# Scthe/cnn-Super-Resolution

Measured on AMD Instinct MI355X. Metric: training tiles/sec (fwd+bwd+update), default SRCNN 33x33, batch 4096/GPU, higher is better.
Workload: dtype f32

## Files before the change

cnn-super-resolution_amd/csrc/hip/d1x6.hpp:

```cpp

constexpr int kD6Mxx = 12, kD6Mx3 = 25;
constexpr int kD6ExWin = 6, kD6ExMid = 3;
constexpr int kD6Grow = 70;

constexpr int kD6Zero = 32;
__device__ __attribute__((aligned(16))) float g_d6_zero[kD6Zero] = {};
constexpr int d6_row_half(bool d3, int h) { return (d3 ? 4 : 8) * h; }
constexpr int d6_zero_half(bool d3, int h) { return d6_row_half(d3, h); }
constexpr int d6_row_quad(bool d3, int k) { return d3 ? 8 * k : 16 * (k >> 1) + 4 * (k & 1); }
constexpr bool d6_zero_row_covers(bool d3) {
  for (int h = 0; h < 2; h++)
    for (int k = 0; k < 4; k++)
      if (d6_zero_half(d3, h) + d6_row_quad(d3, k) + 4 > kD6Zero) return false;
  return true;
}

__device__ __forceinline__ void mma_x6_2(const bf16x8 (&a0)[3], const bf16x8 (&b0)[3], f32x16& c0,
                                         const bf16x8 (&a1)[3], const bf16x8 (&b1)[3], f32x16& c1) {
  using mfma::mma_bf16;
  c0 = mma_bf16(a0[2], b0[0], c0);
  c1 = mma_bf16(a1[2], b1[0], c1);
  c0 = mma_bf16(a0[1], b0[1], c0);
  c1 = mma_bf16(a1[1], b1[1], c1);
  c0 = mma_bf16(a0[0], b0[2], c0);
  c1 = mma_bf16(a1[0], b1[2], c1);
  c0 = mma_bf16(a0[1], b0[0], c0);
  c1 = mma_bf16(a1[1], b1[0], c1);
  c0 = mma_bf16(a0[0], b0[1], c0);
  c1 = mma_bf16(a1[0], b1[1], c1);
  c0 = mma_bf16(a0[0], b0[0], c0);
  c1 = mma_bf16(a1[0], b1[0], c1);
}

__device__ __forceinline__ void d6_split(const float (&v)[8], bf16x8 (&o)[3]) { mfma::split8(v, o); }

template <bool kD3, bool kTr = false>
__global__ __launch_bounds__(256, 1) void d1x6_grad12_kernel(const float* __restrict__ X,
                                                              const float* __restrict__ A1T,
                                                              const float* __restrict__ D2,
                                                              const float* __restrict__ A2,
                                                              const uint32_t* __restrict__ M2,
                                                              const float* __restrict__ W2,
                                                              const float* __restrict__ W3,
                                                              float* __restrict__ slab, Geom g, RunGeom rg,
                                                              D3Geom dg) {
  constexpr int N1 = 64, N2 = 32, F1 = 9, K1 = F1 * F1;
  constexpr int NW1 = K1 * N1, NW2 = N1 * N2, P12 = NW1 + N1 + NW2 + N2;
  extern __shared__ __attribute__((aligned(16))) float smem[];
  static_assert(kD3 || !kTr, "the part images belong to the delta3 form");
  const D6Lds L(g.W, g.H, rg, kD3);
  char* const base = reinterpret_cast<char*>(smem);
  __bf16* const w2i = reinterpret_cast<__bf16*>(base + L.w2);
  uint32_t* const u32 = reinterpret_cast<uint32_t*>(smem);
  uint32_t* const xbuf = u32 + L.xb / 4;
  int* const slots = reinterpret_cast<int*>(base + L.slots);
  int* const runs = reinterpret_cast<int*>(base + L.runs);

  SRCNN_CLOCK_BEGIN();
  const int lane = mfma::lane_id(), wave = mfma::wave_id();
  const int h = lane >> 5, li = lane & 31;
  const int W = g.W, xn = g.W * g.H, npx = g.ow * g.oh, nch = rg.nch;
  const int x0col = 4 * rg.a;

  float xr[kL12Regs];
  auto xload = [&](int smp) {
    const float* src = X + (size_t)smp * xn;
#pragma unroll
    for (int k = 0; k < kL12Regs; k++) {
      const int i = threadIdx.x + 256 * k;
      xr[k] = i < xn ? src[i] : 0.0f;
    }
  };
  if ((int)blockIdx.x < g.batch) xload(blockIdx.x);

  if constexpr (!kTr)
    for (int i = threadIdx.x; i < nch * 32; i += 256) slots[i] = slot_pixel(rg, i >> 5, i & 31);
  for (int k = threadIdx.x; k < nch * 8; k += 256) {
    int iy, ix;
    bool col;
    run_origin(rg, k < rg.nrun ? k : 0, iy, ix, col);
    runs[(k & ~7) + 4 * (k & 1) + 2 * ((k >> 2) & 1) + ((k >> 1) & 1)] =
        col ? ~(L.rdw + 3 * ((ix - x0col) * L.st + iy)) : 3 * (iy * L.rs + ix);
  }
  for (int i = threadIdx.x; i < (2 * L.xbuf + 3) / 4; i += 256) reinterpret_cast<uint4*>(xbuf)[i] = uint4{0u, 0u, 0u, 0u};
  if (threadIdx.x < 32 && (!kD3 || threadIdx.x < kD6Mxx || (threadIdx.x >= 16 && threadIdx.x < kD6Mx3)))
    u32[L.cst / 4 + threadIdx.x] = !kD3 && (threadIdx.x == 0 || threadIdx.x == 6) ? 0x3F803F80u : 0u;
  {
    constexpr int kIt = 2 * 2 * 64 * 8 / 256;
    float v[kIt];
#pragma unroll
    for (int k = 0; k < kIt; k++) {
      const int e = threadIdx.x + 256 * k;
      const int j = e & 7, L_ = (e >> 3) & 63, kk = (e >> 9) & 1, t = e >> 10;
      const int n = kD3 ? crow(8 * kk + j, L_ >> 5) : 16 * kk + 8 * (L_ >> 5) + j;
      v[k] = W2[(32 * t + (L_ & 31)) * N2 + n];
    }
#pragma unroll
    for (int k = 0; k < kIt; k++) {
      const int e = threadIdx.x + 256 * k;
      const int j = e & 7, L_ = (e >> 3) & 63, kk = (e >> 9) & 1, t = e >> 10;
      __bf16 p[3];
      split3(v[k], p[0], p[1], p[2]);
#pragma unroll
      for (int q = 0; q < 3; q++) w2i[((t * 2 + kk) * 3 + q) * 512 + L_ * 8 + j] = p[q];
    }
  }

  uint32_t* const d3u = u32 + L.d3img / 4;
  const int nout3 = dg.w3 * dg.h3;
  float d3n[2] = {0.0f, 0.0f};
  auto d3load = [&](int smp) {
#pragma unroll
    for (int k = 0; k < 2; k++) {
      const int t = threadIdx.x + 256 * k;
      d3n[k] = t < nout3 ? D2[(size_t)smp * nout3 + t] : 0.0f;
    }
  };
  auto d3build = [&](int buf) {
    uint16_t* const b16 = reinterpret_cast<uint16_t*>(d3u + buf * L.d3buf);
#pragma unroll
    for (int k = 0; k < 2; k++) {
      const int t = threadIdx.x + 256 * k;
      if (t < nout3) {
        const int y = t / dg.w3, x = t - y * dg.w3, d = (y + 5) * L.gs + x + 7;
        __bf16 p[3];
        split3(d3n[k], p[0], p[1], p[2]);
#pragma unroll
        for (int q = 0; q < 3; q++) {
          const uint16_t b = __builtin_bit_cast(uint16_t, p[q]);
          b16[2 * (d + L.gw * q)] = b;
          b16[2 * (d + L.gw * q) - 1] = b;
        }
      }
    }
  };
  float* const mxx = smem + L.cst / 4 + kD6Mxx;
  float* const mx3 = smem + L.cst / 4 + kD6Mx3;
  auto wave_max = [&](float v) {
#pragma unroll
    for (int o = 32; o > 0; o >>= 1) v = fmaxf(v, __shfl_xor(v, o, 64));
    return v;
  };
  auto put_max = [&](float* slot, float v) {
    v = wave_max(v);
    if (lane == 0) slot[wave] = v;
  };
  auto take_max_reg = [&](float v) {
    return __builtin_bit_cast(float, __builtin_amdgcn_readfirstlane(__builtin_bit_cast(int, v)));
  };
  auto take_max = [&](const float* slot) {
    const float v = fmaxf(fmaxf(slot[0], slot[1]), fmaxf(slot[2], slot[3]));
    return __builtin_bit_cast(float, __builtin_amdgcn_readfirstlane(__builtin_bit_cast(int, v)));
  };
  float m3cur = 0.0f, wnorm = 0.0f;
  int EW = 0, EB = 0, EWmin = 1 << 20, EBmin = 1 << 20;
  if constexpr (kD3) {
    {
      float n2 = 0.0f, n3 = 0.0f;
      for (int n = 0; n < N2; n++) n2 += fabsf(W2[lane * N2 + n]);
      for (int t = 0; t < dg.f3 * dg.f3; t++) n3 += fabsf(W3[t * N2 + li]);
      wnorm = take_max_reg(wave_max(n2)) * take_max_reg(wave_max(n3));
    }
    __bf16* const w3i = reinterpret_cast<__bf16*>(base + L.w3i);
    constexpr int kW3It = 2 * 64 * 8 / 256;
    static_assert(kW3It * 256 * 3 == kD6W3, "the W3 image: 2 k-steps x 3 parts");
    float w3v[kW3It];
#pragma unroll
    for (int k = 0; k < kW3It; k++) {
      const int e = threadIdx.x + 256 * k;
      const int j = e & 7, L_ = (e >> 3) & 63, s_ = e >> 9;
      const D3Pair tp = d3_pair_slot(8 * s_ + 4 * (L_ >> 5) + (j >> 1), dg.f3);
      const int dx = d3_pair_dx(tp, j & 1, dg.f3), n = L_ & 31;
      const bool in = dx >= 0;
      w3v[k] = W3[in ? (tp.dy * dg.f3 + dx) * N2 + n : 0];
      if (!in) w3v[k] = 0.0f;
    }
#pragma unroll
    for (int k = 0; k < kW3It; k++) {
      const int e = threadIdx.x + 256 * k;
      const int j = e & 7, L_ = (e >> 3) & 63, s_ = e >> 9;
      __bf16 p[3];
      split3(w3v[k], p[0], p[1], p[2]);
#pragma unroll
      for (int q = 0; q < 3; q++) w3i[((s_ * 3 + q) * 64 + L_) * 8 + j] = p[q];
    }
    int* const d3tab = reinterpret_cast<int*>(base + L.d3tab);
    for (int i = threadIdx.x; i < nch * 32; i += 256) {
      int iy, ix;
      slot_coord(rg, i >> 5, i & 31, iy, ix);
      d3tab[i] = kTr ? d6_slot_pack(slot_pixel(rg, i >> 5, i & 31), iy * L.gs + ix) : iy * L.gs + ix;
    }
    for (int i = threadIdx.x; i < (3 * L.d3buf + 3) / 4; i += 256)
      reinterpret_cast<uint4*>(d3u)[i] = uint4{0u, 0u, 0u, 0u};
    if ((int)blockIdx.x < g.batch) d3load(blockIdx.x);
    put_max(mx3, fmaxf(fabsf(d3n[0]), fabsf(d3n[1])));
    __syncthreads();
    m3cur = take_max(mx3);
    d3build(0);
    if ((int)blockIdx.x + (int)gridDim.x < g.batch) d3load(blockIdx.x + gridDim.x);
  }

  int offR3[3], offT3[3];
#pragma unroll
  for (int u = 0; u < 3; u++) {
    const int tap = 32 * u + li;
    const int dy = tap < K1 ? tap / F1 : 0, dx = tap < K1 ? tap - dy * F1 : 0;
    offR3[u] = 12 * (dy * L.rs + dx);
    offT3[u] = 12 * (dx * L.st + dy);
  }
  typedef __attribute__((address_space(3))) const uint32_t lds_u32;
  const int lds0 = (int)(uintptr_t)(__attribute__((address_space(3))) char*)base;
  const int spec = li == K1 - 64 ? lds0 + L.cst : li > K1 - 64 ? lds0 + L.cst + 64 : -1;

  f32x16 g1[2][3], g2[2];
#pragma unroll
  for (int t = 0; t < 2; t++) {
    g2[t] = zero16();
#pragma unroll
    for (int u = 0; u < 3; u++) g1[t][u] = zero16();
  }
  float gb2 = 0.0f;
  float gbr[16];
#pragma unroll
  for (int r = 0; r < 16; r++) gbr[r] = 0.0f;

  float* const sc = smem + L.sc / 4 + wave * kD6Sc;
  char* const trw = base + L.sc + d6tr_wave_off(wave);
  char* const trw0 = trw + d6tr_write_off(li, h, 0, 0, 0);
  char* const trw1 = trw + d6tr_write_off(li, h, 1, 0, 0);
  const char* const trr = trw + d6tr_read_off(lane, 0, 0, 0);
  const uint16_t* const wl2 = reinterpret_cast<const uint16_t*>(w2i) + lane * 8;

  const float inv_nch = 1.0f / (float)nch;
  auto item = [&](int i, int& j, int& c) {
    j = run_div(i, inv_nch);
    c = i - j * nch;
  };
  auto item_sample = [&](int j) {
    const int smp = (int)blockIdx.x + j * (int)gridDim.x;
    return smp < g.batch ? smp : (int)blockIdx.x;
  };
  f32x4 d2r[4], a1r[2][4];
  uint32_t d2m = 0, d2raw = 0;
  int d2pix = 0;
  auto ld_d2 = [&](int j, int c, int sv) {
    const int pix = kTr ? d6_slot_pix(sv) : slots[c * 32 + li];
    if constexpr (kD3) {
      d2pix = pix;
      d2raw = M2[(size_t)item_sample(j) * npx + (pix >= 0 ? pix : 0)];
    } else {
      static_assert(d6_zero_row_covers(false), "dummy-slot loads past g_d6_zero");
      const float* d2 = pix >= 0 ? D2 + ((size_t)item_sample(j) * npx + pix) * N2 + d6_row_half(false, h)
// ... 118 lines not shown
#pragma unroll
    for (int r = 0; r < 16; r++) {
      const float v = acc[0][r] + acc[1][r];
      d2v[r] = mask_d2(r, v);
    }
  };

  bf16x8 w2k0[2][3];
  auto w2read0 = [&]() __attribute__((always_inline)) {
#pragma unroll
    for (int q = 0; q < 3; q++) {
      w2k0[0][q] = *reinterpret_cast<const bf16x8*>(wl2 + ((0 * 2 + 0) * 3 + q) * 512);
      w2k0[1][q] = *reinterpret_cast<const bf16x8*>(wl2 + ((1 * 2 + 0) * 3 + q) * 512);
    }
  };

  int ki = wave, kj, kc;
  item(ki, kj, kc);
  __syncthreads();
  w2read0();
  {
    const int sv = kD3 ? d3tab_[kc * 32 + li] : 0;
    ld_d2(kj, kc, sv);
    ld_a1(kj, kc);
    if constexpr (kD3) {
      bf16x8 ga[3], gb[3];
      const int t = kTr ? d6_slot_off(sv) : sv;
      d3read(kj, t, 0, ga, gb);
      d2gemm(kj, t, ga, gb);
    } else {
      take_rows();
    }
  }
  if constexpr (kTr) {
    sum_d2(1.0f);
#pragma unroll
    for (int k = 0; k < 2; k++) {
      split_d2(1 + k);
      tr_write(k);
    }
    __builtin_amdgcn_wave_barrier();
    tr_read(0);
    tr_read(1);
  } else {
    stage_d2();
#pragma unroll
    for (int piece = 0; piece < 5; piece++) split_d2(piece);
  }

  for (int it = 0; (int)blockIdx.x + it * (int)gridDim.x < g.batch; it++) {
    const int smp = blockIdx.x + it * gridDim.x;
    uint32_t* const xi = xbuf + (it & 1) * L.xbuf;
    float s1 = 1.0f, sX = 1.0f;
    float m3next = 0.0f;
    if constexpr (kD3) {
      float xm = 0.0f;
#pragma unroll
      for (int k = 0; k < kL12Regs; k++) xm = fmaxf(xm, fabsf(xr[k]));
      float dm = fmaxf(fabsf(d3n[0]), fabsf(d3n[1]));
#pragma unroll
      for (int o = 32; o > 0; o >>= 1) {
        const float tx = __shfl_xor(xm, o, 64), td = __shfl_xor(dm, o, 64);
        xm = fmaxf(xm, tx);
        dm = fmaxf(dm, td);
      }
      if (lane == 0) {
        mxx[wave] = xm;
        mx3[wave] = dm;
      }
      if (smp + (int)gridDim.x < g.batch) d3build((it + 1) - 3 * ((it + 1) / 3));
      __syncthreads();
      const float xmax = take_max(mxx);
      m3next = take_max(mx3);
      const float bound = m3cur * wnorm;
      int e1 = mfma::scale_exp_h(bound), exn = mfma::scale_exp_h(xmax), ex = 0, kb = 0, dW = 0, dB = 0;
      if (exn < mfma::kScaleMin + kD6ExMid) exn = mfma::kScaleMin + kD6ExMid;
      if (bound > 0.0f) {
        int exc = e1 + exn - kD6ExMid - (EWmin + kD6Grow);
        if (exc < e1 - (EBmin + kD6Grow)) exc = e1 - (EBmin + kD6Grow);
        if (exc > 0) e1 = e1 - exc < mfma::kScaleMin ? mfma::kScaleMin : e1 - exc;
        kb = EB - e1;
        if (kb < -14 || kb > 15) {
          dB = e1 - EB;
          EB = e1;
          kb = 0;
        }
        if (xmax > 0.0f) {
          ex = EW - e1;
          if (ex > exn || ex < exn - kD6ExWin) {
            ex = exn - kD6ExMid;
            dW = e1 + ex - EW;
            EW = e1 + ex;
          }
        }
        if (EW < EWmin) EWmin = EW;
        if (EB < EBmin) EBmin = EB;
      } else {
        e1 = 0;
        ex = xmax > 0.0f ? exn - kD6ExMid : 0;
      }
      s1 = mfma::pow2_h(e1);
      sX = mfma::pow2_h(ex);
      if (threadIdx.x == 0) {
        const uint32_t c = (uint32_t)(kb + 15) << 10;
        u32[L.cst / 4 + 3 * (it & 1)] = u32[L.cst / 4 + 3 * (it & 1) + 6] = c | (c << 16);
      }
      while (dW != 0 || dB != 0) {
        const int a = dW < -120 ? -120 : dW > 120 ? 120 : dW, b = dB < -120 ? -120 : dB > 120 ? 120 : dB;
        const float fw = mfma::pow2_h(a), fb = li == K1 - 64 ? mfma::pow2_h(b) : fw;
#pragma unroll
        for (int t = 0; t < 2; t++)
#pragma unroll
          for (int u = 0; u < 3; u++) {
            const float f = u == 2 ? fb : fw;
#pragma unroll
            for (int r = 0; r < 16; r++) g1[t][u][r] *= f;
            __builtin_amdgcn_sched_barrier(0);
          }
        dW -= a;
        dB -= b;
      }
    }
    if constexpr (kD3) {
      uint16_t* const x16 = reinterpret_cast<uint16_t*>(xi);
#pragma unroll
      for (int k = 0; k < kL12Regs; k++) {
        const int i = threadIdx.x + 256 * k;
        if (i < xn) {
          const float xs = xr[k] * sX;
          const _Float16 p0 = (_Float16)xs;
          const _Float16 p[2] = {p0, (_Float16)(xs - (float)p0)};
          const int y = i / W, x = i - y * W, ri = y * L.rs + x;
          const int ti = L.rdw + 3 * ((x - x0col) * L.st + y);
#pragma unroll
          for (int q = 0; q < 2; q++) {
            const uint16_t b = __builtin_bit_cast(uint16_t, p[q]);
            x16[2 * (3 * ri + q)] = b;
            if (ri > 0) x16[2 * (3 * (ri - 1) + q) + 1] = b;
            if (L.tcols && x >= x0col) {
              x16[2 * (ti + q)] = b;
              if (y > 0) x16[2 * (ti - 3 + q) + 1] = b;
            }
          }
        }
      }
    } else {
      uint16_t* const x16 = reinterpret_cast<uint16_t*>(xi);
#pragma unroll
      for (int k = 0; k < kL12Regs; k++) {
        const int i = threadIdx.x + 256 * k;
        if (i < xn) {
          __bf16 p[3];
          split3(xr[k], p[0], p[1], p[2]);
          const int y = i / W, x = i - y * W, ri = y * L.rs + x;
          const int ti = L.rdw + 3 * ((x - x0col) * L.st + y);
#pragma unroll
          for (int q = 0; q < 3; q++) {
            const uint16_t b = __builtin_bit_cast(uint16_t, p[q]);
            x16[2 * (3 * ri + q)] = b;
            if (ri > 0) x16[2 * (3 * (ri - 1) + q) + 1] = b;
            if (L.tcols && x >= x0col) {
              x16[2 * (ti + q)] = b;
              if (y > 0) x16[2 * (ti - 3 + q) + 1] = b;
            }
          }
        }
      }
    }
    __syncthreads();
    const int nsmp = smp + (int)gridDim.x;
    if (nsmp < g.batch) xload(nsmp);
    if constexpr (kD3) {
      if (nsmp + (int)gridDim.x < g.batch) d3load(nsmp + gridDim.x);
    }
    const int xo = L.xb / 4 + (it & 1) * L.xbuf;

    while (kj == it) {
      const int c = kc;
      int nj, nc;
      item(ki + 4, nj, nc);

      if constexpr (!kTr) gb2 += gbs;
      if constexpr (!kD3) ld_d2(nj, nc, 0);
      const u32x4 rc4 = *reinterpret_cast<const u32x4*>(runs + 8 * c + 4 * h);
      int xrb[2][2];
      bool xrt[2][2];
#pragma unroll
      for (int m = 0; m < 2; m++)
#pragma unroll
        for (int e = 0; e < 2; e++) {
          const int code = (int)rc4[2 * m + e];
          xrt[m][e] = code < 0;
          xrb[m][e] = lds0 + 4 * (xo + (code < 0 ? ~code : code));
        }
      const int d3s = kD3 ? d3tab_[nc * 32 + li] : 0;
      const int d3t = kTr ? d6_slot_off(d3s) : d3s;
      __builtin_amdgcn_sched_barrier(0);
      if constexpr (kD3) ld_d2(nj, nc, d3s);
      f32x16 d1[2] = {zero16(), zero16()};
      {
        bf16x8 b0[3], b1[3];
#pragma unroll
        for (int q = 0; q < 3; q++) {
          b0[q] = *reinterpret_cast<const bf16x8*>(wl2 + ((0 * 2 + 1) * 3 + q) * 512);
          b1[q] = *reinterpret_cast<const bf16x8*>(wl2 + ((1 * 2 + 1) * 3 + q) * 512);
        }
        mma_x6_2(da[0], w2k0[0], d1[0], da[0], w2k0[1], d1[1]);
        mma_x6_2(da[1], b0, d1[0], da[1], b1, d1[1]);
      }
      bf16x8 aa[2][2][3];
#pragma unroll
      for (int t = 0; t < 2; t++)
#pragma unroll
        for (int m = 0; m < 2; m++) {
          float v[8];
#pragma unroll
          for (int j = 0; j < 8; j++) v[j] = a1r[t][2 * m + (j >> 2)][j & 3];
          d6_split(v, aa[t][m]);
        }
#pragma unroll
      for (int i = 0; i < 24; i++) {
        __builtin_amdgcn_sched_group_barrier(0x008, 1, 0);
        __builtin_amdgcn_sched_group_barrier(0x002, 7, 0);
        __builtin_amdgcn_sched_group_barrier(0x100, 1, 0);
        if (kD3 && i == 1) __builtin_amdgcn_sched_group_barrier(0x020, 1, 0);
      }
// ... 114 lines not shown
        if constexpr (kD3)
          mfma::mma_x3_h_2(dxh[m][0], bxh[st & 1], g1[0][u], dxh[m][1], bxh[st & 1], g1[1][u]);
        else
          mma_x6_2(dx[m][0], bx[st & 1], g1[0][u], dx[m][1], bx[st & 1], g1[1][u]);
        if (kTr) {
          if (st == 0) {
            mask_take();
#pragma unroll
            for (int r = 0; r < 16; r++) {
              const float v = gacc[0][r] + gacc[1][r];
              d2v[r] = mask_d2(r, v);
            }
          }
          if (st == 1 || st == 2) {
            split_d2(st);
            tr_write(st - 1);
          }
          if (st == 3) {
            sum_d2((int)blockIdx.x + nj * (int)gridDim.x < g.batch ? 1.0f : 0.0f);
            __builtin_amdgcn_wave_barrier();
            tr_read(0);
            tr_read(1);
          }
        } else if (kD3) {
          if (st == 0) {
            mask_take();
#pragma unroll
            for (int r = 0; r < 16; r++) {
              const float v = gacc[0][r] + gacc[1][r];
              d2v[r] = mask_d2(r, v);
            }
            stage_d2();
          }
          if (st == 1) split_d2(0);
          if (st >= 1 && st <= 4) split_d2(st);
        } else if (st < 2) {
          split_d1(1, st);
          if (st == 1) split_d2(0);
        } else {
          split_d2(st - 1);
        }
#pragma unroll
        for (int i = 0; i < (kD3 ? 6 : 12); i++) {
          __builtin_amdgcn_sched_group_barrier(0x008, 1, 0);
          __builtin_amdgcn_sched_group_barrier(0x002, kD3 ? 12 : 6, 0);
          __builtin_amdgcn_sched_group_barrier(0x100, kD3 ? 2 : 1, 0);
        }
        __builtin_amdgcn_sched_barrier(0);
      }
      ki += 4;
      kj = nj;
      kc = nc;
    }
    m3cur = m3next;
  }
  SRCNN_CLOCK_END(g_clk, 2);

  __syncthreads();
  float* const red = smem;
  float* out = slab + (size_t)blockIdx.x * P12;
  float* const stg = smem + 4 * 4 * 16 * 64;
  auto stg_w1 = [&](int row, int ch) -> float& { return stg[row * N1 + (ch ^ ((row & 15) << 2))]; };
  auto tile_ref = [&](int k) -> f32x16& { return k < 6 ? g1[k / 3][k % 3] : g2[k - 6]; };
#pragma unroll
  for (int rd = 0; rd < 2; rd++) {
#pragma unroll
    for (int k = 0; k < 4; k++) {
      const f32x16& a = tile_ref(4 * rd + k);
#pragma unroll
      for (int r = 0; r < 16; r++) red[((k * 4 + wave) * 16 + r) * 64 + lane] = a[r];
    }
    __syncthreads();
#pragma unroll
    for (int k = 0; k < 4; k++) {
      if (wave != k) continue;
      const int tile = 4 * rd + k;
      f32x16 sum;
#pragma unroll
      for (int r = 0; r < 16; r++) {
        float v = red[((k * 4 + 0) * 16 + r) * 64 + lane];
#pragma unroll
        for (int w = 1; w < 4; w++) v += red[((k * 4 + w) * 16 + r) * 64 + lane];
        sum[r] = v;
      }
      if (tile < 6) {
        const int t = tile / 3, u = tile % 3, tap = 32 * u + li;
        if constexpr (kD3) {
          int e = -(tap == K1 ? EB : EW);
#pragma unroll
          for (int k = 0; k < 3; k++) {
            const int a = e < -126 ? -126 : e > 126 ? 126 : e;
            const float f = mfma::pow2_h(a);
#pragma unroll
            for (int r = 0; r < 16; r++) sum[r] *= f;
            e -= a;
          }
        }
#pragma unroll
        for (int r = 0; r < 16; r++)
          if (tap <= K1) stg_w1(tap, 32 * t + crow(r, h)) = sum[r];
      } else {
        const int t = tile - 6;
#pragma unroll
        for (int r = 0; r < 16; r++) stg[NW1 + N1 + (32 * t + crow(r, h)) * N2 + li] = sum[r];
      }
    }
    __syncthreads();
// ... 32 lines not shown
```

cnn-super-resolution_amd/csrc/hip/d3taps.hpp:

```cpp
struct D3Pair {
  int dy;
  int col;
  bool used;
};

__host__ __device__ constexpr D3Pair d3_pair_slot(int p, int f3) {
  const int npr = (f3 + 1) / 2, g = p >> 2, e = p & 3;
  return e < 3 ? D3Pair{g, 2 + 2 * e, g < f3 && 2 - e < npr} : D3Pair{4, 6 - 2 * g, 4 < f3 && g < npr};
}

__host__ __device__ constexpr int d3_pair_dx(D3Pair t, int i, int f3) {
  const int dx = 7 - (t.col + i);
  return t.used && dx >= 0 && dx < f3 ? dx : -1;
}

__host__ __device__ constexpr bool d3_pairs_addressable(int f3) {
  for (int g = 0; g < 4; g++) {
    const D3Pair a = d3_pair_slot(4 * g, f3);
    for (int e = 0; e < 4; e++) {
      const D3Pair t = d3_pair_slot(4 * g + e, f3);
      if (t.dy < 0 || t.dy > 4 || t.col < 0 || t.col > 6) return false;
      if (e < 3 && (t.dy != a.dy || t.col != a.col + 2 * e)) return false;
    }
  }
  return true;
}
static_assert(d3_pairs_addressable(1) && d3_pairs_addressable(2) && d3_pairs_addressable(3) &&
                  d3_pairs_addressable(4) && d3_pairs_addressable(5),
              "d1x6's delta3 reads: one base per row group");
```

cnn-super-resolution_amd/csrc/hip/l12x6.hpp:

```cpp
using mfma::bf16x8;
using mfma::f16x8;
using mfma::mma_x3_h;
using mfma::mma_x6;
using mfma::relu1;
using mfma::split3;
using mfma::split8;
using mfma::split8_h;
using mfma::split8_pk;
using mfma::u32x4;

template <bool kLazy>
__global__ __launch_bounds__(256, 2) void l12x6_fwd_kernel(const float* __restrict__ X,
                                                            const float* __restrict__ W1,
                                                            const float* __restrict__ B1,
                                                            const float* __restrict__ W2,
                                                            const float* __restrict__ B2,
                                                            float* __restrict__ A1,
                                                            float* __restrict__ A2, Geom g, RunGeom rg,
                                                            LazyUpdate lz) {
  constexpr int N1 = 64, N2 = 32, F1 = 9, NT1 = 2;
  extern __shared__ __attribute__((aligned(16))) float smem[];
  const H6Lds L(g.W, g.H);
  _Float16* const w1i = reinterpret_cast<_Float16*>(smem);
  _Float16* const w2i = w1i + kH6W1;
  float* const a88s = reinterpret_cast<float*>(w2i + kH6W2);
  float* const b2i = a88s + 128;
  float* const b2s = b2i + 32;
  float* const wmx = b2s + 32;
  float* const w2mx = wmx + 4;
  float* const xmx = w2mx + 4;
  uint32_t* const rimg = reinterpret_cast<uint32_t*>(reinterpret_cast<char*>(smem) + L.r);
  float* const xs = reinterpret_cast<float*>(reinterpret_cast<char*>(smem) + L.xs);
  const int rs = L.rs;
  float* const a2sc = reinterpret_cast<float*>(reinterpret_cast<char*>(smem) + L.a2sc);

  SRCNN_CLOCK_BEGIN();
  const int lane = mfma::lane_id(), wave = mfma::wave_id();
  const int h = lane >> 5, li = lane & 31;
  const int W = g.W, xn = g.W * g.H;
  const int npx = g.ow * g.oh, nch = rg.nch;

  float xr[kL12Regs];
  auto xload = [&](int smp) {
    const float* src = X + (size_t)smp * xn;
#pragma unroll
    for (int k = 0; k < kL12Regs; k++) {
      const int i = threadIdx.x + 256 * k;
      xr[k] = i < xn ? src[i] : 0.0f;
    }
  };
  if ((int)blockIdx.x < g.batch) xload(blockIdx.x);
  auto wave_max = [&](float v) {
#pragma unroll
    for (int o = 32; o > 0; o >>= 1) v = fmaxf(v, __shfl_xor(v, o, 64));
    return v;
  };
  auto max4 = [&](const float* slot) {
    const f32x4 m = *reinterpret_cast<const f32x4*>(slot);
    return fmaxf(fmaxf(m[0], m[1]), fmaxf(m[2], m[3]));
  };

  if constexpr (kLazy) lazy_write_slice(lz);
  auto prm = [&](int seg, int i) -> float {
    if constexpr (kLazy) return lazy_param(lz, seg, i);
    return (seg == 0 ? W1 : seg == 1 ? B1 : seg == 2 ? W2 : B2)[i];
  };
  auto prm4 = [&](int seg, int i, f32x4& v, f32x4& m, f32x4& gr) {
    if constexpr (kLazy) {
      const uint32_t gi = lz.off[seg] + i;
      v = *reinterpret_cast<const f32x4*>(lz.P + gi);
      m = *reinterpret_cast<const f32x4*>(lz.M + gi);
      gr = *reinterpret_cast<const f32x4*>(lz.G + gi);
    } else {
      v = *reinterpret_cast<const f32x4*>((seg == 0 ? W1 : W2) + i);
    }
  };
  auto upd4 = [&](int seg, f32x4& v, f32x4& m, const f32x4& gr) {
    if constexpr (kLazy) {
#pragma unroll
      for (int e = 0; e < 4; e++) {
        float w_ = v[e], m_ = m[e];
        sgd_step(w_, m_, seg, gr[e], lz.lr[seg >> 1], lz.mu, lz.wd, lz.batch);
        v[e] = w_;
      }
    }
  };
  constexpr int kQ1 = 5120 / 4 / 256, kQ2 = 2048 / 4 / 256;
  f32x4 v1[kQ1], v2[kQ2];
  float a88v = 0.0f, b2v = 0.0f, wm = 0.0f, w2m = 0.0f;
  {
    f32x4 m[kQ1], gr[kQ1];
#pragma unroll
    for (int k = 0; k < kQ1; k++) prm4(0, 4 * (threadIdx.x + 256 * k), v1[k], m[k], gr[k]);
    if (threadIdx.x < 128) a88v = threadIdx.x < 64 ? prm(0, 80 * N1 + threadIdx.x) : prm(1, threadIdx.x - 64);
    if (threadIdx.x < 64) wm = fabsf(a88v);
    f32x4 ns = {0.0f, 0.0f, 0.0f, 0.0f};
#pragma unroll
    for (int k = 0; k < kQ1; k++) {
      upd4(0, v1[k], m[k], gr[k]);
#pragma unroll
      for (int e = 0; e < 4; e++) {
        wm = fmaxf(wm, fabsf(v1[k][e]));
        ns[e] += fabsf(v1[k][e]);
      }
    }
#pragma unroll
    for (int e = 0; e < 4; e++) {
      ns[e] += __shfl_xor(ns[e], 16, 64);
      ns[e] += __shfl_xor(ns[e], 32, 64);
    }
    if (lane < 16) *reinterpret_cast<f32x4*>(a2sc + wave * kX6Sc + 4 * lane) = ns;
  }
  {
    f32x4 m[kQ2], gr[kQ2];
#pragma unroll
    for (int k = 0; k < kQ2; k++) prm4(2, 4 * (threadIdx.x + 256 * k), v2[k], m[k], gr[k]);
#pragma unroll
    for (int k = 0; k < kQ2; k++) {
      upd4(2, v2[k], m[k], gr[k]);
#pragma unroll
      for (int e = 0; e < 4; e++) w2m = fmaxf(w2m, fabsf(v2[k][e]));
    }
  }
  wm = wave_max(wm);
  w2m = wave_max(w2m);
  if (lane == 0) {
    wmx[wave] = wm;
    w2mx[wave] = w2m;
  }
  if (threadIdx.x >= 128 && threadIdx.x < 160) {
    const int i = threadIdx.x - 128;
    b2v = prm(3, crow(i & 15, i >> 4));
  }
  const float a80 = fabsf(prm(0, 80 * N1 + lane)), b1a = fabsf(prm(1, lane));
  __syncthreads();
  const int ew = mfma::scale_exp_h(max4(wmx)), ew2 = mfma::scale_exp_h(max4(w2mx));
  const float wnorm = wave_max(a80 + ((a2sc[lane] + a2sc[kX6Sc + lane]) + (a2sc[2 * kX6Sc + lane] + a2sc[3 * kX6Sc + lane])));
  const float b1max = wave_max(b1a);
  {
    const float sw = mfma::pow2_h(ew);
#pragma unroll
    for (int k = 0; k < kQ1; k++) {
      const int p0 = 4 * (threadIdx.x + 256 * k), tap = p0 >> 6, dy = tap / F1, dx = tap - dy * F1;
      const int gg = dx < 8 ? dy : 9, j = dx < 8 ? dx : dy, s_ = gg >> 1, hh = gg & 1;
#pragma unroll
      for (int e = 0; e < 4; e++) {
        const int ch = (p0 & 63) + e, t = ch >> 5, L_ = (ch & 31) + 32 * hh;
        const float ws_ = v1[k][e] * sw;
        const _Float16 q0 = (_Float16)ws_, q1 = (_Float16)(ws_ - (float)q0);
        w1i[((s_ * 2 + t) * 2 + 0) * 512 + L_ * 8 + j] = q0;
        w1i[((s_ * 2 + t) * 2 + 1) * 512 + L_ * 8 + j] = q1;
      }
    }
    if (threadIdx.x < 128) a88s[threadIdx.x] = a88v * sw;
  }
  {
    const float sw2 = mfma::pow2_h(ew2);
#pragma unroll
    for (int k = 0; k < kQ2; k++) {
      const int p0 = 4 * (threadIdx.x + 256 * k), c = p0 >> 5, r = c & 31;
      const int hh = (r >> 2) & 1, rr = (r & 3) + 4 * (r >> 3), mm = 2 * (c >> 5) + (rr >> 3), j = rr & 7;
#pragma unroll
      for (int e = 0; e < 4; e++) {
        const int L_ = (p0 & 31) + e + 32 * hh;
        const float ws_ = v2[k][e] * sw2;
        const _Float16 q0 = (_Float16)ws_, q1 = (_Float16)(ws_ - (float)q0);
        w2i[(mm * 2 + 0) * 512 + L_ * 8 + j] = q0;
        w2i[(mm * 2 + 1) * 512 + L_ * 8 + j] = q1;
      }
    }
    if (threadIdx.x >= 128 && threadIdx.x < 160) b2i[threadIdx.x - 128] = b2v * sw2;
  }
  __syncthreads();
  float a88r[NT1];
#pragma unroll
  for (int t = 0; t < NT1; t++) a88r[t] = a88s[64 * h + 32 * t + li];

  constexpr int NST = 32 * NT1 / 2 + N2 / 8;
  f32x16 pa1[NT1], pa2 = zero16();
#pragma unroll
  for (int t = 0; t < NT1; t++) pa1[t] = zero16();
  bool pok = false;
  float* pa1p = A1;
  float* pa2p = A2;
  int ppx[4] = {-1, -1, -1, -1};
  auto store_prev = [&](int k) {
    if (pok) {
      if (k < 16 * NT1) {
        const int t = k >> 4, r = k & 15;
        __builtin_nontemporal_store(pa1[t][r], pa1p + (32 * t + crow(r, h)) * 32);
      } else {
        const int q = k - 16 * NT1;
        if (ppx[q] >= 0) {
          f32x4 v_;
#pragma unroll
          for (int e = 0; e < 4; e++) v_[e] = pa2[4 * q + e];
          *reinterpret_cast<f32x4*>(pa2p + (size_t)ppx[q] * N2 + 4 * (lane & 7)) = v_;
        }
      }
    }
  };

  const uint16_t* const wl1 = reinterpret_cast<const uint16_t*>(w1i) + lane * 8;
  const uint16_t* const wl2 = reinterpret_cast<const uint16_t*>(w2i) + lane * 8;
  auto w1op = [&](int s, int t, f16x8 (&a)[2]) {
#pragma unroll
    for (int q = 0; q < 2; q++) a[q] = *reinterpret_cast<const f16x8*>(wl1 + ((s * 2 + t) * 2 + q) * 512);
  };

  for (int sample = blockIdx.x; sample < g.batch; sample += gridDim.x) {
    {
      float xm = 0.0f;
#pragma unroll
      for (int k = 0; k < kL12Regs; k++) xm = fmaxf(xm, fabsf(xr[k]));
      xm = wave_max(xm);
      if (lane == 0) xmx[wave] = xm;
    }
    __syncthreads();
    const int ex = mfma::scale_exp_h(max4(xmx));
    const float sx = mfma::pow2_h(ex);
    const int eu = -(ew + ex), eu1 = eu > 127 ? 127 : eu;
    const float un1 = mfma::pow2_h(eu1), un2 = mfma::pow2_h(eu - eu1);
    const int ea = mfma::scale_exp_h(max4(xmx) * wnorm + b1max);
    const float sa = mfma::pow2_h(ea);
    const int ev = -(ea + ew2), ev1 = ev > 127 ? 127 : ev;
    const float vn1 = mfma::pow2_h(ev1), vn2 = mfma::pow2_h(ev - ev1);
    if (threadIdx.x < 32) b2s[threadIdx.x] = b2i[threadIdx.x] * sa;
    {
      uint16_t* const r16 = reinterpret_cast<uint16_t*>(rimg);
#pragma unroll
      for (int k = 0; k < kL12Regs; k++) {
        const int i = threadIdx.x + 256 * k;
        if (i < xn) {
          const float xv = xr[k] * sx;
          xs[i] = xv;
          const int y = i / W, x = i - y * W, d = y * rs + x;
          const _Float16 q0 = (_Float16)xv, q1 = (_Float16)(xv - (float)q0);
          const uint16_t b0 = __builtin_bit_cast(uint16_t, q0), b1 = __builtin_bit_cast(uint16_t, q1);
          r16[2 * d] = b0;
          r16[2 * (d + W)] = b1;
          if (x > 0) {
            r16[2 * d - 1] = b0;
            r16[2 * (d + W) - 1] = b1;
          }
        }
      }
    }
    __syncthreads();
    if (sample + (int)gridDim.x < g.batch) xload(sample + gridDim.x);

    for (int c = wave; c < nch; c += 4) {
      int iy, ix;
      const bool pv = slot_coord(rg, c, li, iy, ix);
      const int rb = (iy + h) * rs + ix;
      const int b4 = h ? iy * W + ix + 8 : (iy + 8) * W + ix, st4 = h ? W : 1;

      f32x16 acc1[NT1];
      {
        const float bx = h ? sx : xs[(iy + 8) * W + ix + 8];
#pragma unroll
        for (int t = 0; t < NT1; t++) acc1[t] = mma(a88r[t], bx, zero16());
      }
      auto xop = [&](int s, f16x8 (&b)[2]) {
#pragma unroll
        for (int q = 0; q < 2; q++) {
          const uint32_t* r = rimg + W * q + rb + 2 * s * rs;
          u32x4 d;
          d[0] = r[0];
// ... 105 lines not shown
```

cnn-super-resolution_amd/csrc/hip/split.hpp:

```cpp
#pragma once

#include <hip/hip_runtime.h>
#include <stdint.h>

#include "mfma.hpp"

namespace srcnn {
namespace mfma {

typedef __bf16 bf16x8 __attribute__((ext_vector_type(8)));
typedef uint32_t u32x4 __attribute__((ext_vector_type(4)));

__device__ __forceinline__ void split3(float a, __bf16& p0, __bf16& p1, __bf16& p2) {
  p0 = (__bf16)a;
  const float r = a - (float)p0;
  p1 = (__bf16)r;
  p2 = (__bf16)(r - (float)p1);
}

typedef float f32x2 __attribute__((ext_vector_type(2)));
typedef __bf16 bf16x2 __attribute__((ext_vector_type(2)));

__device__ __forceinline__ void split8_pk(const float (&v)[8], bf16x8 (&o)[3]) {
#pragma unroll
// ... 52 lines not shown
  c = mma_bf16(a[1], b[1], c);
  c = mma_bf16(a[0], b[2], c);
  c = mma_bf16(a[1], b[0], c);
  c = mma_bf16(a[0], b[1], c);
  return mma_bf16(a[0], b[0], c);
}

__device__ __forceinline__ f32x4 mma16_bf16(const bf16x8& a, const bf16x8& b, f32x4 c) {
  return __builtin_amdgcn_mfma_f32_16x16x32_bf16(a, b, c, 0, 0, 0);
}

__device__ __forceinline__ f32x4 mma16_x6(const bf16x8 (&a)[3], const bf16x8 (&b)[3], f32x4 c) {
  c = mma16_bf16(a[2], b[0], c);
  c = mma16_bf16(a[1], b[1], c);
  c = mma16_bf16(a[0], b[2], c);
  c = mma16_bf16(a[1], b[0], c);
  c = mma16_bf16(a[0], b[1], c);
  return mma16_bf16(a[0], b[0], c);
}

typedef _Float16 f16x8 __attribute__((ext_vector_type(8)));
typedef _Float16 f16x2 __attribute__((ext_vector_type(2)));

__device__ __forceinline__ void split8_h(const float (&v)[8], f16x8 (&o)[2]) {
#pragma unroll
  for (int j = 0; j < 8; j += 2) {
    const f16x2 p0 = __builtin_convertvector((f32x2){v[j], v[j + 1]}, f16x2);
    const f32x2 h0 = __builtin_convertvector(p0, f32x2);
    const f16x2 p1 = __builtin_convertvector((f32x2){v[j] - h0[0], v[j + 1] - h0[1]}, f16x2);
    o[0][j] = p0[0];
    o[0][j + 1] = p0[1];
    o[1][j] = p1[0];
    o[1][j + 1] = p1[1];
  }
}

__device__ __forceinline__ void split_pair_h(float a, float b, uint32_t (&o)[2]) {
  const f16x2 p0 = __builtin_convertvector((f32x2){a, b}, f16x2);
  const f32x2 h0 = __builtin_convertvector(p0, f32x2);
  const f16x2 p1 = __builtin_convertvector((f32x2){a - h0[0], b - h0[1]}, f16x2);
  o[0] = __builtin_bit_cast(uint32_t, p0);
  o[1] = __builtin_bit_cast(uint32_t, p1);
}

constexpr int kScaleMin = -126, kScaleMax = 60;
__device__ __forceinline__ int scale_exp_h(float bound) {
  const int field = (__builtin_bit_cast(uint32_t, bound) >> 23) & 0xFF;
  if (bound == 0.0f) return 0;
  const int e = 14 - (field - 127);
  return e < kScaleMin ? kScaleMin : e > kScaleMax ? kScaleMax : e;
}
__device__ __forceinline__ float pow2_h(int e) { return __builtin_bit_cast(float, (uint32_t)(e + 127) << 23); }

__device__ __forceinline__ f32x16 mma_f16(const f16x8& a, const f16x8& b, f32x16 c) {
  return __builtin_amdgcn_mfma_f32_32x32x16_f16(a, b, c, 0, 0, 0);
}

__device__ __forceinline__ f32x16 mma_x3_h(const f16x8 (&a)[2], const f16x8 (&b)[2], f32x16 c) {
  c = mma_f16(a[1], b[0], c);
  c = mma_f16(a[0], b[1], c);
  return mma_f16(a[0], b[0], c);
}

__device__ __forceinline__ void mma_x3_h_2(const f16x8 (&a0)[2], const f16x8 (&b0)[2], f32x16& c0,
                                           const f16x8 (&a1)[2], const f16x8 (&b1)[2], f32x16& c1) {
  c0 = mma_f16(a0[1], b0[0], c0);
  c1 = mma_f16(a1[1], b1[0], c1);
  c0 = mma_f16(a0[0], b0[1], c0);
  c1 = mma_f16(a1[0], b1[1], c1);
  c0 = mma_f16(a0[0], b0[0], c0);
  c1 = mma_f16(a1[0], b1[0], c1);
}

}
}
```

Before: 7.056 million.

## Compute next sample's scale exponents a step ahead, drop barrier, use DPP wave max

The per-sample max reduction and scale-exponent computation move one iteration ahead. Input tiles and delta3 for the sample after next are prefetched into a second register set, and the maxima are written to double-buffered (parity-indexed) LDS slots. This removes the dedicated __syncthreads that previously sat between the max reduction and the scale computation in each iteration. The wave max reduction is also replaced by DPP row ops plus readlane instead of shuffles, and the W3 norm loads are unrolled over a fixed tap count. The cost is more registers for the extra prefetch buffers, which could lower occupancy.

```diff
diff --git a/cnn-super-resolution_amd/csrc/hip/d1x6.hpp b/cnn-super-resolution_amd/csrc/hip/d1x6.hpp
--- a/cnn-super-resolution_amd/csrc/hip/d1x6.hpp
+++ b/cnn-super-resolution_amd/csrc/hip/d1x6.hpp
@@ -1,5 +1,15 @@
 
-constexpr int kD6Mxx = 12, kD6Mx3 = 25;
+constexpr int kD6Mxx = 12, kD6MxxPar = 6, kD6Mx3 = 24, kD6Mx3Par = 4;
+constexpr bool d6_cst_image(int t) { return t < 12 || (t & ~1) == 16 || (t & ~1) == 22; }
+constexpr bool d6_cst_slots_clear() {
+  for (int par = 0; par < 2; par++)
+    for (int k = 0; k < 4; k++)
+      if (d6_cst_image(kD6Mxx + kD6MxxPar * par + k) || d6_cst_image(kD6Mx3 + kD6Mx3Par * par + k) ||
+          kD6Mx3 + kD6Mx3Par * par + k >= 32)
+        return false;
+  return true;
+}
+static_assert(d6_cst_slots_clear(), "the maxima's slots lie in the constant region, off its images");
 constexpr int kD6ExWin = 6, kD6ExMid = 3;
 constexpr int kD6Grow = 70;
 
@@ -62,16 +72,35 @@
   const int W = g.W, xn = g.W * g.H, npx = g.ow * g.oh, nch = rg.nch;
   const int x0col = 4 * rg.a;
 
-  float xr[kL12Regs];
-  auto xload = [&](int smp) {
+  float xr[kL12Regs], xq[kL12Regs];
+  if constexpr (kD3) {
+#pragma unroll
+    for (int k = 0; k < kL12Regs; k++) xr[k] = xq[k] = 0.0f;
+  }
+  auto xload = [&](int smp, float (&x)[kL12Regs]) {
     const float* src = X + (size_t)smp * xn;
 #pragma unroll
     for (int k = 0; k < kL12Regs; k++) {
       const int i = threadIdx.x + 256 * k;
-      xr[k] = i < xn ? src[i] : 0.0f;
-    }
-  };
-  if ((int)blockIdx.x < g.batch) xload(blockIdx.x);
+      x[k] = i < xn ? src[i] : 0.0f;
+    }
+  };
+  const int nout3 = dg.w3 * dg.h3;
+  float d3n[2] = {0.0f, 0.0f};
+  auto d3load = [&](int smp, float (&d)[2]) {
+#pragma unroll
+    for (int k = 0; k < 2; k++) {
+      const int t = threadIdx.x + 256 * k;
+      d[k] = t < nout3 ? D2[(size_t)smp * nout3 + t] : 0.0f;
+    }
+  };
+  if ((int)blockIdx.x < g.batch) {
+    xload(blockIdx.x, xr);
+    if constexpr (kD3) d3load(blockIdx.x, d3n);
+  }
+  if constexpr (kD3) {
+    if ((int)blockIdx.x + (int)gridDim.x < g.batch) xload(blockIdx.x + gridDim.x, xq);
+  }
 
   if constexpr (!kTr)
     for (int i = threadIdx.x; i < nch * 32; i += 256) slots[i] = slot_pixel(rg, i >> 5, i & 31);
@@ -83,7 +112,7 @@
         col ? ~(L.rdw + 3 * ((ix - x0col) * L.st + iy)) : 3 * (iy * L.rs + ix);
   }
   for (int i = threadIdx.x; i < (2 * L.xbuf + 3) / 4; i += 256) reinterpret_cast<uint4*>(xbuf)[i] = uint4{0u, 0u, 0u, 0u};
-  if (threadIdx.x < 32 && (!kD3 || threadIdx.x < kD6Mxx || (threadIdx.x >= 16 && threadIdx.x < kD6Mx3)))
+  if (threadIdx.x < 32 && (!kD3 || d6_cst_image(threadIdx.x)))
     u32[L.cst / 4 + threadIdx.x] = !kD3 && (threadIdx.x == 0 || threadIdx.x == 6) ? 0x3F803F80u : 0u;
   {
     constexpr int kIt = 2 * 2 * 64 * 8 / 256;
@@ -107,15 +136,6 @@
   }
 
   uint32_t* const d3u = u32 + L.d3img / 4;
-  const int nout3 = dg.w3 * dg.h3;
-  float d3n[2] = {0.0f, 0.0f};
-  auto d3load = [&](int smp) {
-#pragma unroll
-    for (int k = 0; k < 2; k++) {
-      const int t = threadIdx.x + 256 * k;
-      d3n[k] = t < nout3 ? D2[(size_t)smp * nout3 + t] : 0.0f;
-    }
-  };
   auto d3build = [&](int buf) {
     uint16_t* const b16 = reinterpret_cast<uint16_t*>(d3u + buf * L.d3buf);
 #pragma unroll
@@ -136,13 +156,8 @@
   };
   float* const mxx = smem + L.cst / 4 + kD6Mxx;
   float* const mx3 = smem + L.cst / 4 + kD6Mx3;
-  auto wave_max = [&](float v) {
-#pragma unroll
-    for (int o = 32; o > 0; o >>= 1) v = fmaxf(v, __shfl_xor(v, o, 64));
-    return v;
-  };
   auto put_max = [&](float* slot, float v) {
-    v = wave_max(v);
+    v = mfma::wave_max(v);
     if (lane == 0) slot[wave] = v;
   };
   auto take_max_reg = [&](float v) {
@@ -152,14 +167,57 @@
     const float v = fmaxf(fmaxf(slot[0], slot[1]), fmaxf(slot[2], slot[3]));
     return __builtin_bit_cast(float, __builtin_amdgcn_readfirstlane(__builtin_bit_cast(int, v)));
   };
-  float m3cur = 0.0f, wnorm = 0.0f;
+  float wnorm = 0.0f;
   int EW = 0, EB = 0, EWmin = 1 << 20, EBmin = 1 << 20;
+  float s1n = 1.0f, sXn = 1.0f;
+  int kbn = 0, dWn = 0, dBn = 0;
+  auto scales = [&](float m3, float xmax) __attribute__((always_inline)) {
+    const float bound = m3 * wnorm;
+    int e1 = mfma::scale_exp_h(bound), exn = mfma::scale_exp_h(xmax), ex = 0, kb = 0, dW = 0, dB = 0;
+    if (exn < mfma::kScaleMin + kD6ExMid) exn = mfma::kScaleMin + kD6ExMid;
+    if (bound > 0.0f) {
+      int exc = e1 + exn - kD6ExMid - (EWmin + kD6Grow);
+      if (exc < e1 - (EBmin + kD6Grow)) exc = e1 - (EBmin + kD6Grow);
+      if (exc > 0) e1 = e1 - exc < mfma::kScaleMin ? mfma::kScaleMin : e1 - exc;
+      kb = EB - e1;
+      if (kb < -14 || kb > 15) {
+        dB = e1 - EB;
+        EB = e1;
+        kb = 0;
+      }
+      if (xmax > 0.0f) {
+        ex = EW - e1;
+        if (ex > exn || ex < exn - kD6ExWin) {
+          ex = exn - kD6ExMid;
+          dW = e1 + ex - EW;
+          EW = e1 + ex;
+        }
+      }
+      if (EW < EWmin) EWmin = EW;
+      if (EB < EBmin) EBmin = EB;
+    } else {
+      e1 = 0;
+      ex = xmax > 0.0f ? exn - kD6ExMid : 0;
+    }
+    s1n = mfma::pow2_h(e1);
+    sXn = mfma::pow2_h(ex);
+    kbn = kb;
+    dWn = dW;
+    dBn = dB;
+  };
   if constexpr (kD3) {
     {
-      float n2 = 0.0f, n3 = 0.0f;
+      float n2 = 0.0f, n3 = 0.0f, w3a[kD3MaxTaps];
+#pragma unroll
+      for (int t = 0; t < kD3MaxTaps; t++) {
+        const bool in = t < dg.f3 * dg.f3;
+        w3a[t] = fabsf(W3[(in ? t : 0) * N2 + li]);
+        if (!in) w3a[t] = 0.0f;
+      }
       for (int n = 0; n < N2; n++) n2 += fabsf(W2[lane * N2 + n]);
-      for (int t = 0; t < dg.f3 * dg.f3; t++) n3 += fabsf(W3[t * N2 + li]);
-      wnorm = take_max_reg(wave_max(n2)) * take_max_reg(wave_max(n3));
+#pragma unroll
+      for (int t = 0; t < kD3MaxTaps; t++) n3 += w3a[t];
+      wnorm = take_max_reg(mfma::wave_max(n2)) * take_max_reg(mfma::wave_max(n3));
     }
     __bf16* const w3i = reinterpret_cast<__bf16*>(base + L.w3i);
     constexpr int kW3It = 2 * 64 * 8 / 256;
@@ -192,12 +250,23 @@
     }
     for (int i = threadIdx.x; i < (3 * L.d3buf + 3) / 4; i += 256)
       reinterpret_cast<uint4*>(d3u)[i] = uint4{0u, 0u, 0u, 0u};
-    if ((int)blockIdx.x < g.batch) d3load(blockIdx.x);
+    float d3q[2] = {0.0f, 0.0f};
+    if ((int)blockIdx.x + (int)gridDim.x < g.batch) d3load(blockIdx.x + gridDim.x, d3q);
+    {
+      float xm = 0.0f;
+#pragma unroll
+      for (int k = 0; k < kL12Regs; k++) xm = fmaxf(xm, fabsf(xr[k]));
+      put_max(mxx, xm);
+    }
     put_max(mx3, fmaxf(fabsf(d3n[0]), fabsf(d3n[1])));
     __syncthreads();
-    m3cur = take_max(mx3);
+    {
+      const float xmax = take_max(mxx), m3 = take_max(mx3);
+      if ((int)blockIdx.x < g.batch) scales(m3, xmax);
+    }
     d3build(0);
-    if ((int)blockIdx.x + (int)gridDim.x < g.batch) d3load(blockIdx.x + gridDim.x);
+    d3n[0] = d3q[0];
+    d3n[1] = d3q[1];
   }
 
   int offR3[3], offT3[3];
@@ -422,59 +491,25 @@
     const int smp = blockIdx.x + it * gridDim.x;
     uint32_t* const xi = xbuf + (it & 1) * L.xbuf;
     float s1 = 1.0f, sX = 1.0f;
-    float m3next = 0.0f;
+    [[maybe_unused]] const bool more = smp + (int)gridDim.x < g.batch;
     if constexpr (kD3) {
       float xm = 0.0f;
 #pragma unroll
-      for (int k = 0; k < kL12Regs; k++) xm = fmaxf(xm, fabsf(xr[k]));
+      for (int k = 0; k < kL12Regs; k++) xm = fmaxf(xm, fabsf(xq[k]));
       float dm = fmaxf(fabsf(d3n[0]), fabsf(d3n[1]));
-#pragma unroll
-      for (int o = 32; o > 0; o >>= 1) {
-        const float tx = __shfl_xor(xm, o, 64), td = __shfl_xor(dm, o, 64);
-        xm = fmaxf(xm, tx);
-        dm = fmaxf(dm, td);
-      }
+      xm = mfma::wave_max(xm);
+      dm = mfma::wave_max(dm);
       if (lane == 0) {
-        mxx[wave] = xm;
-        mx3[wave] = dm;
-      }
-      if (smp + (int)gridDim.x < g.batch) d3build((it + 1) - 3 * ((it + 1) / 3));
-      __syncthreads();
-      const float xmax = take_max(mxx);
-      m3next = take_max(mx3);
-      const float bound = m3cur * wnorm;
-      int e1 = mfma::scale_exp_h(bound), exn = mfma::scale_exp_h(xmax), ex = 0, kb = 0, dW = 0, dB = 0;
-      if (exn < mfma::kScaleMin + kD6ExMid) exn = mfma::kScaleMin + kD6ExMid;
-      if (bound > 0.0f) {
-        int exc = e1 + exn - kD6ExMid - (EWmin + kD6Grow);
-        if (exc < e1 - (EBmin + kD6Grow)) exc = e1 - (EBmin + kD6Grow);
-        if (exc > 0) e1 = e1 - exc < mfma::kScaleMin ? mfma::kScaleMin : e1 - exc;
-        kb = EB - e1;
-        if (kb < -14 || kb > 15) {
-          dB = e1 - EB;
-          EB = e1;
-          kb = 0;
-        }
-        if (xmax > 0.0f) {
-          ex = EW - e1;
-          if (ex > exn || ex < exn - kD6ExWin) {
-            ex = exn - kD6ExMid;
-            dW = e1 + ex - EW;
-            EW = e1 + ex;
-          }
-        }
-        if (EW < EWmin) EWmin = EW;
-        if (EB < EBmin) EBmin = EB;
-      } else {
-        e1 = 0;
-        ex = xmax > 0.0f ? exn - kD6ExMid : 0;
-      }
-      s1 = mfma::pow2_h(e1);
-      sX = mfma::pow2_h(ex);
+        mxx[kD6MxxPar * ((it + 1) & 1) + wave] = xm;
+        mx3[kD6Mx3Par * ((it + 1) & 1) + wave] = dm;
+      }
+      s1 = s1n;
+      sX = sXn;
       if (threadIdx.x == 0) {
-        const uint32_t c = (uint32_t)(kb + 15) << 10;
+        const uint32_t c = (uint32_t)(kbn + 15) << 10;
         u32[L.cst / 4 + 3 * (it & 1)] = u32[L.cst / 4 + 3 * (it & 1) + 6] = c | (c << 16);
       }
+      int dW = dWn, dB = dBn;
       while (dW != 0 || dB != 0) {
         const int a = dW < -120 ? -120 : dW > 120 ? 120 : dW, b = dB < -120 ? -120 : dB > 120 ? 120 : dB;
         const float fw = mfma::pow2_h(a), fb = li == K1 - 64 ? mfma::pow2_h(b) : fw;
@@ -490,6 +525,7 @@
         dW -= a;
         dB -= b;
       }
+      if (more) d3build((it + 1) - 3 * ((it + 1) / 3));
     }
     if constexpr (kD3) {
       uint16_t* const x16 = reinterpret_cast<uint16_t*>(xi);
@@ -539,9 +575,17 @@
     }
     __syncthreads();
     const int nsmp = smp + (int)gridDim.x;
-    if (nsmp < g.batch) xload(nsmp);
     if constexpr (kD3) {
-      if (nsmp + (int)gridDim.x < g.batch) d3load(nsmp + gridDim.x);
+      const float xmax = take_max(mxx + kD6MxxPar * ((it + 1) & 1)), m3 = take_max(mx3 + kD6Mx3Par * ((it + 1) & 1));
+      if (more) scales(m3, xmax);
+#pragma unroll
+      for (int k = 0; k < kL12Regs; k++) xr[k] = xq[k];
+      if (nsmp + (int)gridDim.x < g.batch) {
+        xload(nsmp + gridDim.x, xq);
+        d3load(nsmp + gridDim.x, d3n);
+      }
+    } else {
+      if (nsmp < g.batch) xload(nsmp, xr);
     }
     const int xo = L.xb / 4 + (it & 1) * L.xbuf;
 
@@ -762,7 +806,6 @@
       kj = nj;
       kc = nc;
     }
-    m3cur = m3next;
   }
   SRCNN_CLOCK_END(g_clk, 2);
 
diff --git a/cnn-super-resolution_amd/csrc/hip/d3taps.hpp b/cnn-super-resolution_amd/csrc/hip/d3taps.hpp
--- a/cnn-super-resolution_amd/csrc/hip/d3taps.hpp
+++ b/cnn-super-resolution_amd/csrc/hip/d3taps.hpp
@@ -3,6 +3,8 @@
   int col;
   bool used;
 };
+
+constexpr int kD3MaxTaps = 25;
 
 __host__ __device__ constexpr D3Pair d3_pair_slot(int p, int f3) {
   const int npr = (f3 + 1) / 2, g = p >> 2, e = p & 3;
diff --git a/cnn-super-resolution_amd/csrc/hip/l12x6.hpp b/cnn-super-resolution_amd/csrc/hip/l12x6.hpp
--- a/cnn-super-resolution_amd/csrc/hip/l12x6.hpp
+++ b/cnn-super-resolution_amd/csrc/hip/l12x6.hpp
@@ -50,11 +50,6 @@
     }
   };
   if ((int)blockIdx.x < g.batch) xload(blockIdx.x);
-  auto wave_max = [&](float v) {
-#pragma unroll
-    for (int o = 32; o > 0; o >>= 1) v = fmaxf(v, __shfl_xor(v, o, 64));
-    return v;
-  };
   auto max4 = [&](const float* slot) {
     const f32x4 m = *reinterpret_cast<const f32x4*>(slot);
     return fmaxf(fmaxf(m[0], m[1]), fmaxf(m[2], m[3]));
@@ -122,8 +117,8 @@
       for (int e = 0; e < 4; e++) w2m = fmaxf(w2m, fabsf(v2[k][e]));
     }
   }
-  wm = wave_max(wm);
-  w2m = wave_max(w2m);
+  wm = mfma::wave_max(wm);
+  w2m = mfma::wave_max(w2m);
   if (lane == 0) {
     wmx[wave] = wm;
     w2mx[wave] = w2m;
@@ -135,8 +130,8 @@
   const float a80 = fabsf(prm(0, 80 * N1 + lane)), b1a = fabsf(prm(1, lane));
   __syncthreads();
   const int ew = mfma::scale_exp_h(max4(wmx)), ew2 = mfma::scale_exp_h(max4(w2mx));
-  const float wnorm = wave_max(a80 + ((a2sc[lane] + a2sc[kX6Sc + lane]) + (a2sc[2 * kX6Sc + lane] + a2sc[3 * kX6Sc + lane])));
-  const float b1max = wave_max(b1a);
+  const float wnorm = mfma::wave_max(a80 + ((a2sc[lane] + a2sc[kX6Sc + lane]) + (a2sc[2 * kX6Sc + lane] + a2sc[3 * kX6Sc + lane])));
+  const float b1max = mfma::wave_max(b1a);
   {
     const float sw = mfma::pow2_h(ew);
 #pragma unroll
@@ -213,7 +208,7 @@
       float xm = 0.0f;
 #pragma unroll
       for (int k = 0; k < kL12Regs; k++) xm = fmaxf(xm, fabsf(xr[k]));
-      xm = wave_max(xm);
+      xm = mfma::wave_max(xm);
       if (lane == 0) xmx[wave] = xm;
     }
     __syncthreads();
diff --git a/cnn-super-resolution_amd/csrc/hip/split.hpp b/cnn-super-resolution_amd/csrc/hip/split.hpp
--- a/cnn-super-resolution_amd/csrc/hip/split.hpp
+++ b/cnn-super-resolution_amd/csrc/hip/split.hpp
@@ -128,6 +128,23 @@
 }
 __device__ __forceinline__ float pow2_h(int e) { return __builtin_bit_cast(float, (uint32_t)(e + 127) << 23); }
 
+template <int kCtrl>
+__device__ __forceinline__ float dpp_max(float v) {
+  const int o = __builtin_amdgcn_update_dpp(0, __builtin_bit_cast(int, v), kCtrl, 0xF, 0xF, false);
+  return fmaxf(v, __builtin_bit_cast(float, o));
+}
+__device__ __forceinline__ float wave_max(float v) {
+  v = dpp_max<0xB1>(v);
+  v = dpp_max<0x4E>(v);
+  v = dpp_max<0x141>(v);
+  v = dpp_max<0x140>(v);
+  const int b = __builtin_bit_cast(int, v);
+  float r[4];
+#pragma unroll
+  for (int k = 0; k < 4; k++) r[k] = __builtin_bit_cast(float, __builtin_amdgcn_readlane(b, 16 * k));
+  return fmaxf(fmaxf(r[0], r[1]), fmaxf(r[2], r[3]));
+}
+
 __device__ __forceinline__ f32x16 mma_f16(const f16x8& a, const f16x8& b, f32x16 c) {
   return __builtin_amdgcn_mfma_f32_32x32x16_f16(a, b, c, 0, 0, 0);
 }
```

Result: no change. 7.114 million (median of 6 runs) (+0.8%).
